# zuston/TonY

Measured on AMD Instinct MI355X. Metric: images/sec (whole node) Inception-v3 TF-PS, higher is better.
Workload: dtype bf16

## Files before the change

### tony_amd/ops/_lib.py

```python
from __future__ import annotations

import ctypes
import os
import threading
import weakref
from typing import Dict

import torch

_HERE = os.path.dirname(os.path.abspath(__file__))
SO_PATH = os.environ.get("TONY_KERNELS_SO") or os.path.join(_HERE, "_tony_kernels.so")

_lock = threading.Lock()
_lib = None

c_void_p = ctypes.c_void_p
c_int = ctypes.c_int
c_int64 = ctypes.c_int64
c_float = ctypes.c_float
c_int_p = ctypes.POINTER(ctypes.c_int)
c_void_pp = ctypes.POINTER(ctypes.c_void_p)
c_u8_p = ctypes.POINTER(ctypes.c_uint8)
c_u64_p = ctypes.POINTER(ctypes.c_uint64)

# ... 20 lines not shown
                               c_void_p, c_int64, c_int64, c_int64, c_int64, c_void_p, c_int64, c_int64, c_int,
                               c_void_p, c_void_p, c_void_p, c_void_p, c_int, c_int, c_void_p, c_void_p, c_int64,
                               c_void_p, c_void_p, c_int, c_void_p],
    "tony_bn_relu_maxpool": [c_void_p, c_int64, c_void_p, c_void_p, c_int64, c_void_p, c_void_p, c_int, c_float,
                             c_void_p, c_void_p, c_void_p, c_void_p, c_float, c_void_p, c_int64, c_void_p, c_int,
                             c_int, c_int, c_int, c_int, c_int, c_int, c_void_p],
    "tony_bn_bwd_reduce": [c_void_p, c_int64, c_void_p, c_int64, c_int64, c_int, c_void_p, c_void_p, c_void_p,
                           c_void_p, c_int, c_int, c_void_p, c_void_p, c_int64, c_void_p],
    "tony_bn_bwd_apply": [c_void_p, c_int64, c_void_p, c_int64, c_void_p, c_int64, c_int64, c_int, c_void_p,
                          c_void_p, c_void_p, c_void_p, c_int, c_int, c_void_p, c_void_p, c_int64, c_void_p,
                          c_void_p, c_int, c_void_p],
    "tony_bn_apply_f32_x3": [c_void_p, c_int64, c_int, c_int64, c_void_p, c_int64, c_void_p, c_void_p, c_int64,
                             c_void_p, c_void_p, c_int, c_float, c_int, c_int, c_void_p, c_void_p, c_void_p, c_void_p,
                             c_float, c_void_p],
    "tony_bn_apply_res": [c_void_p, c_int64, c_int, c_int64, c_void_p, c_int64, c_void_p, c_int64, c_void_p,
                          c_void_p, c_int64, c_void_p, c_void_p, c_int, c_float, c_int, c_int, c_void_p, c_void_p,
                          c_void_p, c_void_p, c_float, c_void_p],
    "tony_bn_apply_res_m": [c_void_p, c_int64, c_int, c_int64, c_void_p, c_int64, c_void_p, c_int64, c_void_p,
                            c_void_p, c_int64, c_void_p, c_void_p, c_int, c_float, c_int, c_int, c_void_p, c_void_p,
                            c_void_p, c_void_p, c_float, c_void_p, c_int64, c_void_p],
    "tony_bn_bwd_res": [c_void_p, c_int64, c_void_p, c_int64, c_void_p, c_int64, c_void_p, c_int64, c_void_p, c_int64,
                        c_int64, c_int, c_void_p, c_void_p, c_void_p, c_void_p, c_int, c_void_p, c_void_p, c_void_p,
                        c_int, c_void_p],
    "tony_bn_bwd_res_m": [c_void_p, c_int64, c_void_p, c_int64, c_void_p, c_int64, c_void_p, c_int64, c_void_p,
                          c_int64, c_int64, c_int, c_void_p, c_void_p, c_void_p, c_void_p, c_int, c_void_p, c_void_p,
                          c_void_p, c_int, c_void_p],
    "tony_bn_bwd_onepass": [c_void_p, c_int64, c_void_p, c_int64, c_void_p, c_int64, c_int64, c_int, c_void_p,
                            c_void_p, c_void_p, c_void_p, c_int, c_int, c_void_p, c_void_p, c_void_p, c_int,
                            c_void_p, c_int, c_void_p],
    "tony_add_f32": [c_void_p, c_int, c_void_p, c_int64, c_void_p],
    "tony_sgd_step": [c_void_p, c_void_p, c_void_p, c_int, c_void_p, c_int64, c_void_p, c_void_p],
    "tony_adam_step": [c_void_p, c_void_p, c_void_p, c_void_p, c_int, c_void_p, c_int64, c_void_p, c_void_p],
    "tony_grad_stats": [c_void_p, c_int, c_int64, c_void_p, c_void_p],
    "tony_xent_fwd": [c_void_p, c_int, c_int64, c_int, c_int64, c_void_p, c_float, c_void_p, c_void_p, c_void_p],
    "tony_xent_bwd": [c_void_p, c_int, c_int64, c_int, c_int64, c_void_p, c_float, c_void_p, c_void_p, c_void_p,
                      c_int64, c_void_p],
    "tony_dropout_fwd": [c_void_p, c_void_p, c_void_p, c_int64, c_int, c_float, c_void_p, c_void_p],
    "tony_dropout_bwd": [c_void_p, c_void_p, c_void_p, c_int64, c_int, c_float, c_void_p],
    "tony_counter_bump": [c_void_p, c_void_p],
    "tony_gemm_bf16": [c_void_p, c_void_p, c_void_p, c_int64, c_int64, c_int64, c_int64, c_int64, c_int64,
                       c_int, c_void_p, c_int64, c_void_p],
    "tony_gemm_bf16_bnact": [c_void_p, c_void_p, c_void_p, c_int64, c_int64, c_int64, c_int64, c_int64, c_int64,
                             c_int, c_void_p, c_int64, c_void_p, c_void_p],
    "tony_gemm_tn_bf16": [c_void_p, c_void_p, c_void_p, c_int64, c_int64, c_int64, c_int64, c_int64, c_int64,
                          c_void_p, c_int64, c_void_p, c_int, c_void_p, c_void_p, c_int, c_void_p],
    "tony_splitk_reduce": [c_void_p, c_int, c_int64, c_void_p, c_int, c_int, c_int, c_void_p],
    "tony_splitk_workspace": [c_void_p, c_int64, c_void_p, c_int64],
    "tony_conv_fwd": [c_void_p, c_int, c_int, c_int, c_int, c_int64, c_void_p, c_int, c_int, c_int, c_int, c_int,
                      c_int, c_int, c_void_p, c_int, c_int, c_int64, c_int, c_void_p, c_int64, c_void_p],
    "tony_stem_fwd": [c_void_p, c_int, c_int, c_int, c_int, c_void_p, c_int, c_int, c_int, c_int, c_int, c_int,
                      c_int, c_void_p, c_int, c_int, c_int64, c_int, c_void_p, c_int64, c_int, c_void_p],
    "tony_stem_wgrad": [c_void_p, c_int64, c_void_p, c_int, c_int, c_int, c_int, c_int, c_int, c_int, c_int, c_int,
                        c_int, c_int, c_int, c_int, c_void_p, c_int64, c_void_p, c_int, c_void_p],
    "tony_conv_dgrad": [c_void_p, c_int, c_int, c_int, c_int, c_int64, c_void_p, c_int, c_int, c_int, c_int, c_int,
                        c_void_p, c_int, c_int, c_int64, c_int, c_void_p, c_void_p],
    "tony_conv_dgrad_strided": [c_void_p, c_int, c_int, c_int, c_int, c_int64, c_void_p, c_int, c_int, c_int, c_int,
                                c_int, c_int, c_int, c_void_p, c_int, c_int, c_int64, c_int, c_void_p, c_void_p],
    "tony_conv_wgrad": [c_void_p, c_int64, c_void_p, c_int, c_int, c_int, c_int, c_int64, c_int, c_int, c_int, c_int,
                        c_int, c_int, c_int, c_int, c_int, c_void_p, c_void_p, c_int64, c_void_p, c_int, c_void_p,
                        c_void_p, c_int, c_void_p],
    "tony_conv_wgrad_x3": [c_void_p, c_int64, c_void_p, c_int, c_int, c_int, c_int, c_int64, c_int, c_int, c_int,
                           c_int, c_int, c_int, c_int, c_int, c_int, c_int, c_int, c_void_p, c_int64, c_void_p, c_int,
                           c_void_p],
    "tony_x3_wgrad_mode": [c_int],
    "tony_dgrad_one_launch": [c_int],
    "tony_wgrad_pf": [c_int],
    "tony_kv_copy_blocks": [c_int64],
    "tony_kv_copy_flag": [c_void_p, c_void_p, c_int64, c_void_p, c_void_p],
    "tony_kv_wait": [c_void_p, ctypes.c_uint32, c_void_p, ctypes.c_double, c_void_p],
    "tony_conv_wgrad_direct": [c_void_p, c_int64, c_void_p, c_int, c_int, c_int, c_int, c_int64, c_int, c_int, c_int,
                               c_int, c_int, c_void_p, c_int64, c_void_p, c_int, c_void_p],
    "tony_avgpool3_s1p1": [c_void_p, c_void_p, c_int, c_int, c_int, c_int, c_int64, c_int64, c_void_p],
    "tony_maxpool_fwd": [c_void_p, c_void_p, c_void_p, c_int, c_int, c_int, c_int, c_int, c_int, c_int, c_int64, c_int64,
                         c_void_p],
    "tony_maxpool_bwd": [c_void_p, c_void_p, c_void_p, c_int, c_int, c_int, c_int, c_int, c_int, c_int, c_int64, c_int64,
                         c_void_p],
    "tony_bn_bwd_pool_apply": [c_void_p, c_int64, c_void_p, c_int, c_int, c_int, c_int, c_int, c_int, c_int, c_void_p,
                               c_int64, c_void_p, c_int64, c_void_p, c_void_p, c_void_p, c_void_p, c_int, c_int,
                               c_void_p, c_int64, c_void_p, c_void_p, c_int, c_void_p],
    "tony_maxpool_bwd_acc": [c_void_p, c_void_p, c_void_p, c_int, c_int, c_int, c_int, c_int, c_int, c_int, c_int64, c_int64,
                         c_void_p],
    "tony_maxpool_bwd_bnred": [c_void_p, c_void_p, c_void_p, c_int, c_int, c_int, c_int, c_int, c_int, c_int, c_int64,
                               c_int64, c_void_p, c_int64, c_void_p, c_void_p, c_void_p, c_void_p, c_int, c_int,
                               c_void_p, c_int64, c_int, c_void_p],
    "tony_avgpool_fwd": [c_void_p, c_void_p, c_int, c_int, c_int, c_int, c_int, c_int, c_int64, c_int64, c_void_p],
    "tony_avgpool_bwd": [c_void_p, c_void_p, c_int, c_int, c_int, c_int, c_int, c_int, c_int64, c_int64, c_void_p],
    "tony_transpose_desc_bytes": [],
    "tony_x3_desc_bytes": [],
    "tony_x3_weights_batch": [c_void_p, c_int, c_int, c_void_p],
    "tony_transpose_batch": [c_void_p, c_int, c_int, c_void_p],
    "tony_event_pool": [c_int, c_u64_p],
    "tony_fork": [c_void_p, c_void_p, c_void_p],
    "tony_bn_stats_f32": [c_void_p, c_int64, c_int, c_int64, c_void_p, c_void_p, c_int64, c_void_p],
    "tony_bn_apply_f32": [c_void_p, c_int64, c_int, c_int64, c_void_p, c_int64, c_void_p, c_void_p, c_int64, c_void_p,
                      c_void_p, c_int, c_float, c_int, c_int, c_void_p, c_void_p, c_void_p, c_void_p, c_float,
                      c_void_p],
    "tony_bn_bwd_reduce_f32": [c_void_p, c_int64, c_void_p, c_int64, c_int64, c_int, c_void_p, c_void_p, c_void_p,
                           c_void_p, c_int, c_int, c_void_p, c_void_p, c_int64, c_void_p],
    "tony_bn_bwd_apply_f32": [c_void_p, c_int64, c_void_p, c_int64, c_void_p, c_int64, c_int64, c_int, c_void_p,
                          c_void_p, c_void_p, c_void_p, c_int, c_int, c_void_p, c_void_p, c_int64, c_void_p,
                          c_void_p, c_int, c_void_p],
    "tony_bn_bwd_apply_f32_x3": [c_void_p, c_int64, c_void_p, c_int64, c_void_p, c_int64, c_int64, c_int, c_void_p,
                          c_void_p, c_void_p, c_void_p, c_int, c_int, c_void_p, c_void_p, c_int64, c_void_p,
                          c_void_p, c_int, c_void_p],
    "tony_bn_bwd_apply_f32_x3p": [c_void_p, c_int64, c_void_p, c_int64, c_void_p, c_int64, c_int64, c_int64, c_int,
                                  c_void_p, c_void_p, c_void_p, c_void_p, c_int, c_int, c_void_p, c_void_p, c_int64,
# ... 286 lines not shown
```

### tony_amd/ops/conv.py

```python
from __future__ import annotations

import ctypes
import os
import weakref
from typing import Callable, Dict, Tuple

import torch

from . import _lib, concat, streams, tape, tune, wt_cache
from .arena import zeros_f32
from .bn import HOST_MEMO, _accum_ok, _as_rows, _rows_view
from .gemm import occ_choices, splitk_combine, wgrad_cus, wgrad_tn

_BF16 = torch.bfloat16
AUTOTUNE = os.environ.get("TONY_CONV_AUTOTUNE", "1") != "0"
_CHOICE: Dict[Tuple, str] = {}


def _pair(v):
    if type(v) is tuple:
        return v
    return tuple(v) if isinstance(v, (tuple, list)) else (int(v), int(v))


# ... 77 lines not shown
            return y
    if x.shape[1] < 8:
        return stem_fwd(x, weight, stride, padding, stats)
    key0 = (x.shape, x.stride(), x.dtype, x.device, weight.shape, weight.stride(), weight.dtype, stride, padding,
            stats is not None)
    x, (_, C, ldx) = _as_rows(x)
    n, _, h, w = x.shape
    co, _, r, s = weight.shape
    _lib.check_stat_buffer(stats, co)
    (sh, sw), (ph, pw) = _pair(stride), _pair(padding)
    oh, ow = out_hw(h, w, r, s, stride, padding)
    y = _cl_empty(n, co, oh, ow, x.device)
    wk = _krsc(weight)
    L, st = _lib.lib(), _lib.stream_ptr(x.device)

    def launch(vf, stats_t):
        return L.tony_conv_fwd(x.data_ptr(), n, h, w, C, ldx, wk.data_ptr(), co, r, s, sh, sw, ph, pw, y.data_ptr(),
                               oh, ow, co, (1 if stats_t is not None else 0) | vf, _lib.ptr(stats_t), 2 * co, st)

    if vflags is None:
        key = ("conv_fwd", tuple(x.shape), ldx, tuple(weight.shape), (sh, sw), (ph, pw), stats is not None)
        vflags = tune.cached(key)
        if vflags is None:
            scratch = torch.zeros(_lib.stat_floats(co), device=x.device) if stats is not None else None
            vflags = tune.pick(key, lambda vf: launch(vf, scratch), tune.CONV_VARIANTS)
        if (HOST_MEMO and key0[1] == x.stride() and x.dtype == _BF16 and weight.dtype == _BF16
                and not torch.cuda.is_current_stream_capturing()):
            _FWD_PLAN[key0] = (n, h, w, C, ldx, co, r, s, sh, sw, ph, pw, oh, ow, vflags)
    _lib.check(launch(vflags, stats), "tony_conv_fwd")
    return y


_FWD_PLAN: Dict[Tuple, Tuple] = {}


def stem_fwd(x: torch.Tensor, weight: torch.Tensor, stride=1, padding=0, stats: torch.Tensor | None = None):
    if not stem_supported(x, weight, stride, padding):
        raise ValueError(f"stem_fwd: unsupported conv x={tuple(x.shape)} w={tuple(weight.shape)}")
    n, c, h, w = x.shape
    co, _, r, s = weight.shape
    _lib.check_stat_buffer(stats, co)
    (sh, sw), (ph, pw) = _pair(stride), _pair(padding)
    oh, ow = out_hw(h, w, r, s, stride, padding)
    y = _cl_empty(n, co, oh, ow, x.device)
    wk = _krsc(weight)
    rc = _lib.lib().tony_stem_fwd(x.data_ptr(), n, h, w, c, wk.data_ptr(), co, r, s, sh, sw, ph, pw, y.data_ptr(),
                                  oh, ow, co, 1 if stats is not None else 0, _lib.ptr(stats),
                                  2 * co if stats is not None else 0, _lib.num_cus(x.device),
                                  _lib.stream_ptr(x.device))
    _lib.check(rc, "tony_stem_fwd")
    return y


def stem_wgrad(dy: torch.Tensor, x: torch.Tensor, weight_shape, stride=1, padding=0, dst=None):
    dy, (_, co, lddy) = _as_rows(dy)
    n, c, h, w = x.shape
    _, _, r, s = weight_shape
    (sh, sw), (ph, pw) = _pair(stride), _pair(padding)
    L, dev = _lib.lib(), x.device
    cus = _lib.num_cus(dev)
    nel = co * r * s * c
    slab = torch.empty(2 * cus * nel, dtype=torch.float32, device=dev)
    splits = ctypes.c_int(0)
    st = _lib.stream_ptr(dev)
    rc = L.tony_stem_wgrad(dy.data_ptr(), lddy, x.data_ptr(), n, h, w, c, co, r, s, sh, sw, ph, pw, dy.shape[2],
                           dy.shape[3], slab.data_ptr(), slab.numel(), ctypes.addressof(splits), cus, st)
    _lib.check(rc, "tony_stem_wgrad")
    out = dst if dst is not None else torch.empty(nel, dtype=torch.float32, device=dev)
    rc = L.tony_splitk_reduce(slab.data_ptr(), splits.value, nel, out.data_ptr(), int(out.dtype == _BF16),
                              int(dst is not None), cus, st)
    _lib.check(rc, "tony_splitk_reduce")
    return None if dst is not None else out.view(co, r, s, c).permute(0, 3, 1, 2)


STRIDED_GLDS = os.environ.get("TONY_STRIDED_GLDS", "1") != "0"


def dgrad_supported(x_shape, weight: torch.Tensor, stride=1, padding=0) -> bool:
    (sh, sw), (ph, pw) = _pair(stride), _pair(padding)
    r, s = weight.shape[2], weight.shape[3]
    return x_shape[1] % 8 == 0 and 1 <= sh <= 4 and 1 <= sw <= 4 and 0 <= ph < r and 0 <= pw < s


def conv_dgrad(dy: torch.Tensor, weight: torch.Tensor, x_shape, stride=1, padding=0,
               vflags: int | None = None, bnr: "_lib.BnRed | None" = None,
               accum: torch.Tensor | None = None) -> torch.Tensor:
    if not dgrad_supported(x_shape, weight, stride, padding):
        raise ValueError(f"conv_dgrad: unsupported x={tuple(x_shape)} w={tuple(weight.shape)} stride={stride} "
                         f"padding={padding}")
    n, c, h, w = x_shape
    co, _, r, s = weight.shape
    dy, (_, _, lddy) = _as_rows(dy)
    (sh, sw), (ph, pw) = _pair(stride), _pair(padding)
    dx = _cl_empty(n, c, h, w, dy.device)
    wt = wt_cache.transposed(weight)
    L, st = _lib.lib(), _lib.stream_ptr(dy.device)

    if (sh, sw) == (1, 1):
        def launch(vf, br=None):
            return L.tony_conv_dgrad(dy.data_ptr(), n, dy.shape[2], dy.shape[3], co, lddy, wt.data_ptr(), c, r, s, ph,
                                     pw, dx.data_ptr(), h, w, c, vf, None if br is None else ctypes.addressof(br), st)
        name = "tony_conv_dgrad"
    else:
        def launch(vf, br=None):
            if (vf >> 8) & 0xff in (9, 10, tune.BAND_CODE):
                return -3
            if not STRIDED_GLDS and (vf >> 8) & 0xff >= 11:
                return -3
            return L.tony_conv_dgrad_strided(dy.data_ptr(), n, dy.shape[2], dy.shape[3], co, lddy, wt.data_ptr(), c,
                                             r, s, sh, sw, ph, pw, dx.data_ptr(), h, w, c, vf,
                                             None if br is None else ctypes.addressof(br), st)
        name = "tony_conv_dgrad_strided"

    vf = vflags if vflags is not None else tune.pick(("conv_dgrad", tuple(dy.shape), lddy, tuple(weight.shape),
                                                         (sh, sw), (ph, pw)), launch, tune.CONV_VARIANTS)
    if accum is not None and bnr is None and _accum_ok(accum, x_shape):
        dx = accum
        rc = launch(vf | 16)
        if rc == -3 and (vf >> 8) & 0xff in (9, 10, tune.BAND_CODE):
            rc = launch((vf & ~0xfff00) | 16)
# ... 260 lines not shown
    impl = _choose(key, cands)
    return conv_dgrad(dy, weight, x_shape, stride, padding, bnr=bnr) if impl == "tony" else \
        _miopen_dgrad(dy, weight, x_shape, stride, padding)


MIOPEN_WGRAD_WEIGHT = float(os.environ.get("TONY_MIOPEN_WGRAD_WEIGHT", "1.6"))
WGRAD_IMPL = os.environ.get("TONY_WGRAD_IMPL", "")


def _wgrad(dy, x, weight, stride, padding):
    key = ("wgrad", tuple(dy.shape), tuple(weight.shape), stride, padding)
    impl = _CHOICE.get(key) or WGRAD_IMPL or None
    if fullcover(x.shape, weight.shape, stride, padding):
        impl = "gemm"
        _CHOICE.setdefault(key, impl)
    elif x.shape[1] % 8:
        impl = "stem" if STEM and stem_supported(x, weight, stride, padding) else "miopen"
        _CHOICE.setdefault(key, impl)
    if impl is None:
        impl = _choose(key, {"tony": lambda: conv_wgrad(dy, x, weight.shape, stride, padding),
                             "miopen": lambda: _miopen_wgrad(dy, x, weight, stride, padding)},
                       weight={"miopen": MIOPEN_WGRAD_WEIGHT if streams.ENABLED else 1.0})
    gw = _lib.grad_slot(weight)
    if impl == "gemm":
        if gw is not None and gw.is_contiguous(memory_format=torch.channels_last):
            return streams.run(lambda: _gemm_wgrad(dy, x, weight.shape, dst=gw), dy, x)
        return _accumulate_wgrad(weight, _gemm_wgrad(dy, x, weight.shape))
    if impl == "stem":
        if gw is not None and gw.is_contiguous(memory_format=torch.channels_last):
            return streams.run(lambda: stem_wgrad(dy, x, weight.shape, stride, padding, dst=gw), dy, x)
        return _accumulate_wgrad(weight, stem_wgrad(dy, x, weight.shape, stride, padding))
    if impl == "tony":
        if gw is not None and gw.is_contiguous(memory_format=torch.channels_last):
            return streams.run(lambda: conv_wgrad(dy, x, weight.shape, stride, padding, dst=gw), dy, x)
        return _accumulate_wgrad(weight, conv_wgrad(dy, x, weight.shape, stride, padding))
    if gw is None:
        return _miopen_wgrad(dy, x, weight, stride, padding)

    def into_slot():
        gw.add_(_miopen_wgrad(dy, x, weight, stride, padding))

    return streams.run(into_slot, dy, x)


def _accumulate_wgrad(weight, dw32):
    gw = _lib.grad_slot(weight)
    if gw is None:
        return dw32.to(weight.dtype)
    src = dw32 if gw.is_contiguous(memory_format=torch.channels_last) else dw32.contiguous()
    rc = _lib.lib().tony_add_f32(gw.data_ptr(), int(gw.dtype == _BF16), src.data_ptr(), src.numel(),
                                 _lib.stream_ptr(weight.device))
    _lib.check(rc, "tony_add_f32")
    return None


class _ConvFn(torch.autograd.Function):
    @staticmethod
    def forward(ctx, x, weight, stride, padding):
        y = _fwd(x, weight, stride, padding, None)
        ctx.save_for_backward(x, weight)
        ctx.params = (weight,)
        ctx.stride, ctx.padding = stride, padding
        ctx.bnc_in = getattr(x, "_tony_bnr", None)
        return y

    @staticmethod
    def backward(ctx, dy):
        x, weight = ctx.saved_tensors
        dy = _as_rows(dy)[0]
        dw = _wgrad(dy, x, weight, ctx.stride, ctx.padding)
        dx = _dgrad_fused_bn(ctx, dy, weight, x.shape, ctx.stride, ctx.padding) if ctx.needs_input_grad[0] else None
        streams.keep(dx)
        _lib.report_inplace(ctx.params, (dw,))
        return dx, dw, None, None


def conv2d(x, weight, stride=1, padding=0):
    if supported(x, weight, stride, padding):
        return tape.apply(_ConvFn, x, weight, _pair(stride), _pair(padding))
    if x.is_cuda:
        _record_unsupported("fwd", x.shape, weight.shape, stride, padding)
    return torch.nn.functional.conv2d(x, weight, None, stride, padding)


class _ConvBNActFn(torch.autograd.Function):

    @staticmethod
    def forward(ctx, x, weight, gamma, beta, running_mean, running_var, stride, padding, training, momentum, eps,
                relu, slot=None):
        L = _lib.lib()
        _lib.check_f32_stats(running_mean, running_var)
        dev = x.device
        stream = _lib.stream_ptr(dev)
        co = weight.shape[0]
        stats = zeros_f32(_lib.stat_floats(co), dev) if training else None
        Z = _fwd(x, weight, stride, padding, stats)
        M, _, ldz = _rows_view(Z)
        y = concat.take(slot, *Z.shape, Z)
        if y is None:
            y = torch.empty_like(Z)
        _, _, ldy = _rows_view(y)
        pb = int(gamma.dtype == _BF16)
        if training:
            mean = torch.empty(co, dtype=torch.float32, device=dev)
            invstd = torch.empty(co, dtype=torch.float32, device=dev)
        else:
            mean = running_mean
            invstd = torch.rsqrt(running_var.float() + eps)
        rc = L.tony_bn_apply(Z.data_ptr(), M, co, ldz, y.data_ptr(), ldy, _lib.ptr(stats),
                             _lib.ptr(stats) + 4 * co if training else 0, 2 * co if training else 0,
                             gamma.data_ptr(), beta.data_ptr(), pb,
                             float(eps), int(relu), 0 if training else 1, _lib.ptr(mean) if training else 0,
                             _lib.ptr(invstd) if training else 0, _lib.ptr(running_mean), _lib.ptr(running_var),
                             float(momentum), stream)
        _lib.check(rc, "tony_bn_apply")
        ctx.save_for_backward(x, weight, gamma, beta, mean, invstd, Z)
        ctx.params = (weight, gamma, beta)
        ctx.cfg = (stride, padding, relu, pb)
        ctx.bnc_in = getattr(x, "_tony_bnr", None)
        ctx.join = getattr(x, "_tony_join", None)
        ctx.bnc_self = None
        if training and slot is None:
            ctx.bnc_self = BnCtx(Z, ldz, mean, invstd, gamma, beta, pb, relu)
            y._tony_bnr = ctx.bnc_self
        return y

    @staticmethod
    def backward(ctx, dy):
        x, weight, gamma, beta, mean, invstd, Z = ctx.saved_tensors
        dx, dw, dgamma, dbeta = _conv_bn_backward(ctx, x, weight, gamma, beta, mean, invstd, Z, dy)
        return dx, dw, dgamma, dbeta, None, None, None, None, None, None, None, None, None


def _bn_grad_slots(ctx, gamma, beta):
    gg, gb = _lib.grad_slot(ctx.params[1]), _lib.grad_slot(ctx.params[2])
    inplace = gg is not None and gb is not None
    return (gg if inplace else torch.empty_like(gamma)), (gb if inplace else torch.empty_like(beta)), inplace


def _conv_bn_backward(ctx, x, weight, gamma, beta, mean, invstd, Z, dy, presums=None, done=None):
    stride, padding, relu, pb = ctx.cfg
    dev = x.device
    if done is not None:
        dZ, dgamma, dbeta, inplace = done
    else:
        M, co, ldz = _rows_view(Z)
        if presums is None:
            presums = _bn_presums(ctx, dy)
        dy, (_, _, lddy) = _as_rows(dy)
        dZ = torch.empty_like(Z)
        ws = None if presums is not None else zeros_f32(_lib.bn_bwd_ws_floats(co), dev)
        dgamma, dbeta, inplace = _bn_grad_slots(ctx, gamma, beta)
        _lib.bn_bwd(Z, ldz, dy, lddy, dZ, ldz, M, co, mean, invstd, gamma, beta, pb, relu, ws, dgamma, dbeta, inplace,
                    dev, sums=presums)
    dw = _wgrad(dZ, x, weight, stride, padding)
    join = getattr(ctx, "join", None) if ctx.needs_input_grad[0] else None
    pend = join.take() if join is not None else None
    if pend is not None:
        dx = _dgrad(dZ, weight, x.shape, stride, padding, accum=pend)
    else:
        dx = _dgrad_fused_bn(ctx, dZ, weight, x.shape, stride, padding) if ctx.needs_input_grad[0] else None
        if join is not None:
            dx = join.settle(dx)
    streams.keep(dx)
    if inplace:
        dgamma = dbeta = None
    _lib.report_inplace(ctx.params, (dw, dgamma, dbeta))
    return dx, dw, dgamma, dbeta


class _ConvBNActPoolFn(torch.autograd.Function):

    @staticmethod
    def forward(ctx, x, weight, gamma, beta, running_mean, running_var, stride, padding, momentum, eps, k, s, p=0):
        L = _lib.lib()
        _lib.check_f32_stats(running_mean, running_var)
        dev = x.device
        co = weight.shape[0]
        stats = zeros_f32(_lib.stat_floats(co), dev)
        Z = _fwd(x, weight, stride, padding, stats)
        _, _, ldz = _rows_view(Z)
        n, _, h, w = Z.shape
        oh, ow = (h + 2 * p - k) // s + 1, (w + 2 * p - k) // s + 1
        y = _cl_empty(n, co, oh, ow, dev)
        arg = torch.empty((n, oh, ow, co), dtype=torch.uint8, device=dev)
        mean = torch.empty(co, dtype=torch.float32, device=dev)
        invstd = torch.empty(co, dtype=torch.float32, device=dev)
        pb = int(gamma.dtype == _BF16)
        rc = L.tony_bn_relu_maxpool(Z.data_ptr(), ldz, stats.data_ptr(), stats.data_ptr() + 4 * co, 2 * co,
                                    gamma.data_ptr(), beta.data_ptr(), pb, float(eps), mean.data_ptr(),
                                    invstd.data_ptr(), _lib.ptr(running_mean), _lib.ptr(running_var), float(momentum),
                                    y.data_ptr(), co, arg.data_ptr(), n, h, w, co, k, s, p, _lib.stream_ptr(dev))
        _lib.check(rc, "tony_bn_relu_maxpool")
        ctx.save_for_backward(x, weight, gamma, beta, mean, invstd, Z, arg)
        ctx.params = (weight, gamma, beta)
        ctx.cfg = (stride, padding, True, pb)
        ctx.pool = (k, s, p)
        ctx.bnc_in = getattr(x, "_tony_bnr", None)
        return y

    @staticmethod
    def backward(ctx, dyp):
        x, weight, gamma, beta, mean, invstd, Z, arg = ctx.saved_tensors
        k, s, p = ctx.pool
        n, co, h, w = Z.shape
# ... 101 lines not shown
```

### tony_amd/ops/csrc/bn_act.hip

```cpp
#include <algorithm>
#include <cstdlib>

#include "common.h"

using namespace tony;

namespace {

constexpr int kThreads = 256;
constexpr int kMaxC = 2048;
extern __shared__ __attribute__((aligned(16))) float bn_dyn[];
inline size_t bn_lds_table(int C, int rows) { return static_cast<size_t>(rows) * C * sizeof(float); }
inline size_t bn_lds_reduce(int C) {
  return static_cast<size_t>(2) * (kThreads / (C / 8)) * C * sizeof(float);
}
inline size_t bn_lds_bred(int C) { return std::max(bn_lds_table(C, 4), bn_lds_reduce(C)); }

struct RowMap {
  int CG, RPI, cg, rsub;
  bool active;
  __device__ RowMap(int C) {
    CG = C >> 3;
    RPI = kThreads / CG;
    cg = threadIdx.x % CG;
    rsub = threadIdx.x / CG;
    active = rsub < RPI;
  }
};

struct Segs {
  int n = 0;
  int end[4] = {0, 0, 0, 0};
  void* p[4] = {nullptr, nullptr, nullptr, nullptr};
  int64_t ld[4] = {0, 0, 0, 0};
  template <class T>
  __device__ __forceinline__ void resolve(int col, T*& base, int64_t& ld_out) const {
    int s = 0, start = 0;
    while (s + 1 < n && col >= end[s]) {
      start = end[s];
      ++s;
    }
    base = static_cast<T*>(p[s]) + (col - start);
    ld_out = ld[s];
  }
};

__device__ __forceinline__ float load_param(const void* p, int idx, int is_bf16, float dflt) {
  if (p == nullptr) return dflt;
  return is_bf16 ? bf2f(static_cast<const uint16_t*>(p)[idx]) : static_cast<const float*>(p)[idx];
}

__device__ __forceinline__ void store_param(void* p, int idx, int is_bf16, float v, int accumulate) {
  if (p == nullptr) return;
  if (is_bf16) {
    uint16_t* q = static_cast<uint16_t*>(p) + idx;
    *q = f2bf(accumulate ? bf2f(*q) + v : v);
  } else {
    float* q = static_cast<float*>(p) + idx;
    *q = accumulate ? *q + v : v;
  }
}

__device__ __forceinline__ void block_reduce_add(float* red, const RowMap& rm, int C,
                                                 const float* a, const float* b, float* out_a, float* out_b) {
  if (rm.active) {
#pragma unroll
    for (int j = 0; j < 8; ++j) {
      red[rm.rsub * C + rm.cg * 8 + j] = a[j];
      red[rm.RPI * C + rm.rsub * C + rm.cg * 8 + j] = b[j];
    }
  }
  __syncthreads();
  for (int c = threadIdx.x; c < C; c += kThreads) {
    float sa = 0.f, sb = 0.f;
    for (int k = 0; k < rm.RPI; ++k) {
      sa += red[k * C + c];
      sb += red[rm.RPI * C + k * C + c];
    }
    atomicAdd(out_a + c, sa);
    atomicAdd(out_b + c, sb);
  }
}

template <class T>
__global__ __launch_bounds__(kThreads) void bn_fwd_stats_kernel(
    const T* __restrict__ x, int64_t M, int C, int64_t ldx, int64_t rows_per_block,
    float* __restrict__ sum, float* __restrict__ sumsq, int64_t sstride) {
  float* red = bn_dyn;
  RowMap rm(C);
  float s[8], q[8];
#pragma unroll
  for (int j = 0; j < 8; ++j) s[j] = q[j] = 0.f;
  const int64_t r0 = static_cast<int64_t>(blockIdx.x) * rows_per_block;
  const int64_t r1 = min(M, r0 + rows_per_block);
  if (rm.active) {
    const T* base = x + rm.cg * 8;
    int64_t r = r0 + rm.rsub;
    const int64_t step = rm.RPI;
    for (; r + 3 * step < r1; r += 4 * step) {
      V8<T> v[4];
#pragma unroll
      for (int u = 0; u < 4; ++u) v[u] = V8<T>::load(base + (r + u * step) * ldx);
#pragma unroll
      for (int u = 0; u < 4; ++u) {
        float f[8];
        v[u].to_float(f);
#pragma unroll
        for (int j = 0; j < 8; ++j) {
          s[j] += f[j];
          q[j] = fmaf(f[j], f[j], q[j]);
        }
      }
    }
    for (; r < r1; r += step) {
// ... 1113 lines not shown
```

### tony_amd/ops/csrc/common.h

```cpp
#pragma once
#include <hip/hip_runtime.h>
#include <stdint.h>

#define TONY_API extern "C" __attribute__((visibility("default")))

namespace tony {

static constexpr int kWave = 64;

static constexpr int kStatShards = 8;

__device__ __forceinline__ float shard_sum(const float* p, int c, int64_t sstride) {
  if (sstride == 0) return p[c];
  float s = 0.f;
#pragma unroll
  for (int k = 0; k < kStatShards; ++k) s += p[k * sstride + c];
  return s;
}

__device__ __forceinline__ int64_t shard_off(int idx, int64_t sstride) {
  return sstride == 0 ? 0 : static_cast<int64_t>(idx % kStatShards) * sstride;
}

__device__ __forceinline__ float relu_f(float t) { return t < 0.f ? 0.f : t; }

__device__ __forceinline__ float bf2f(uint16_t v) {
  return __uint_as_float(static_cast<uint32_t>(v) << 16);
}

__device__ __forceinline__ uint16_t f2bf(float f) {
  __bf16 b = static_cast<__bf16>(f);
  return __builtin_bit_cast(uint16_t, b);
}

struct bf16x8 {
  uint4 raw;
  __device__ __forceinline__ void to_float(float* f) const {
    const uint32_t w[4] = {raw.x, raw.y, raw.z, raw.w};
#pragma unroll
    for (int i = 0; i < 4; ++i) {
      f[2 * i] = __uint_as_float(w[i] << 16);
      f[2 * i + 1] = __uint_as_float(w[i] & 0xffff0000u);
    }
  }
  __device__ __forceinline__ static bf16x8 from_float(const float* f) {
    bf16x8 r;
    uint32_t w[4];
#pragma unroll
    for (int i = 0; i < 4; ++i) {
      w[i] = static_cast<uint32_t>(f2bf(f[2 * i])) |
             (static_cast<uint32_t>(f2bf(f[2 * i + 1])) << 16);
    }
    r.raw = make_uint4(w[0], w[1], w[2], w[3]);
    return r;
  }
};

__device__ __forceinline__ bf16x8 load8(const uint16_t* p) {
  bf16x8 r;
  r.raw = *reinterpret_cast<const uint4*>(p);
  return r;
}
__device__ __forceinline__ void store8(uint16_t* p, const bf16x8& v) {
  *reinterpret_cast<uint4*>(p) = v.raw;
}

template <class T>
struct V8;
template <>
struct V8<uint16_t> {
  bf16x8 b;
  __device__ __forceinline__ static V8 load(const uint16_t* p) { return V8{load8(p)}; }
  __device__ __forceinline__ void store(uint16_t* p) const { store8(p, b); }
  __device__ __forceinline__ void to_float(float* f) const { b.to_float(f); }
  __device__ __forceinline__ static V8 from_float(const float* f) { return V8{bf16x8::from_float(f)}; }
};
template <>
struct V8<float> {
  float4 lo, hi;
  __device__ __forceinline__ static V8 load(const float* p) {
    return V8{*reinterpret_cast<const float4*>(p), *reinterpret_cast<const float4*>(p + 4)};
  }
  __device__ __forceinline__ void store(float* p) const {
    *reinterpret_cast<float4*>(p) = lo;
    *reinterpret_cast<float4*>(p + 4) = hi;
// ... 30 lines not shown
```

### tony_amd/ops/csrc/stem.hip

```cpp
#include <type_traits>
#include "mfma_common.h"

using namespace tony;
using namespace tony::mfma;

namespace {

constexpr int kBM = 256;
constexpr int kPatch = 12288;
constexpr int kPF = kPatch / 8 / kThreads;
constexpr int kMaxKSteps = 8;

struct StemGeom {
  const uint16_t* x;
  int H, W, C;
  int R, S, sh, sw, ph, pw;
  int OH, OW;
  int M;
  int K;
  int64_t total;
  float inv_ohw, inv_ow;
};

__device__ __forceinline__ int fast_div(int a, int b, float inv_b) {
// ... 168 lines not shown
#pragma unroll
        for (int i = 0; i < TM; ++i) {
          uint16_t v[8];
#pragma unroll
          for (int e = 0; e < 8; ++e) v[e] = tap_value<NP>(g, src, px[i], tp[e]);
          const bf16x8_t af = pack8(v);
#pragma unroll
          for (int j = 0; j < TN; ++j)
            acc[i][j] = __builtin_amdgcn_mfma_f32_16x16x32_bf16(af, bfr[j], acc[i][j], 0, 0, 0);
        }
      }
    };
    if (staged)
      body(smem);
    else
      body(g.x);
    __syncthreads();
#pragma unroll
    for (int j = 0; j < TN; ++j)
#pragma unroll
      for (int i = 0; i < TM; ++i)
#pragma unroll
        for (int r = 0; r < 4; ++r) {
          const float a = acc[i][j][r];
          ssum[j] += a;
          ssq[j] = fmaf(a, a, ssq[j]);
          smem[(wave * 64 + i * 16 + kq * 4 + r) * LDC + j * 16 + (lane & 15)] = f2bf(a);
        }
    __syncthreads();
    constexpr int CH = BN / 8;
    for (int v = threadIdx.x; v < kBM * CH; v += kThreads) {
      const int row = v / CH, ch = v - row * CH;
      if (m0 + row < g.M)
        *reinterpret_cast<uint4*>(y + static_cast<int64_t>(m0 + row) * ldy + ch * 8) =
            *reinterpret_cast<const uint4*>(smem + row * LDC + ch * 8);
    }
  }
  if (stats == nullptr) return;
  float* st = stats + shard_off(blockIdx.x, sstride);
#pragma unroll
  for (int j = 0; j < TN; ++j) {
    float a = ssum[j], q = ssq[j];
    a += __shfl_xor(a, 16, 64);
    a += __shfl_xor(a, 32, 64);
    q += __shfl_xor(q, 16, 64);
    q += __shfl_xor(q, 32, 64);
    if (lane < 16) {
      atomicAdd(st + j * 16 + lane, a);
      atomicAdd(st + BN + j * 16 + lane, q);
    }
  }
}

template <int CO, int KB, bool NP>
__global__ __launch_bounds__(kThreads) void stem_wgrad_kernel(StemGeom g, const uint16_t* __restrict__ dy,
                                                              int64_t lddy, float* __restrict__ slab, int64_t n) {
  constexpr int PD = CO + 4;
  constexpr int CB = CO / 16;
  constexpr int KW = KB * 16;
  constexpr int DYL = kBM * PD;
  constexpr int RED = CO * KW;
  constexpr int DV = kBM * CO / 8 / kThreads;
  static_assert(RED * 4 <= (DYL + kPatch) * 2, "the fold tile reuses the staging buffers");
  __shared__ __attribute__((aligned(16))) uint16_t smem[DYL + kPatch];
  uint16_t* dyl = smem;
  uint16_t* patch = smem + DYL;

  const int lane = threadIdx.x & 63, wave = threadIdx.x >> 6;
  const int kq = lane >> 4;
  const int kcol0 = blockIdx.y * KW;
  const int kbn = min(KB, (g.K - kcol0 + 15) / 16);
  uint32_t tp[KB];
#pragma unroll
  for (int b = 0; b < KB; ++b) tp[b] = tap_word(g, kcol0 + b * 16 + (lane & 15));

  f32x4 acc[CB][KB];
#pragma unroll
  for (int i = 0; i < CB; ++i)
#pragma unroll
    for (int j = 0; j < KB; ++j) acc[i][j] = f32x4{0.f, 0.f, 0.f, 0.f};

  const int nchunks = (g.M + kBM - 1) / kBM;
  RowPrefetch pf;
  uint4 dv[DV];
  auto issue = [&](int chunk) {
    const int m0 = chunk * kBM, rows = min(kBM, g.M - m0);
    pf.issue(g, m0, m0 + rows - 1);
#pragma unroll
    for (int i = 0; i < DV; ++i) {
      const int v = i * kThreads + threadIdx.x, r = v / (CO / 8), c8 = v % (CO / 8);
      dv[i] = r < rows ? *reinterpret_cast<const uint4*>(dy + static_cast<int64_t>(m0 + r) * lddy + c8 * 8)
                       : make_uint4(0u, 0u, 0u, 0u);
    }
  };
  if (blockIdx.x < nchunks) issue(blockIdx.x);
  for (int chunk = blockIdx.x; chunk < nchunks; chunk += gridDim.x) {
    const int m0 = chunk * kBM;
    __syncthreads();
#pragma unroll
    for (int i = 0; i < DV; ++i) {
      const int v = i * kThreads + threadIdx.x, r = v / (CO / 8), c8 = v % (CO / 8);
      uint2* d = reinterpret_cast<uint2*>(dyl + r * PD + c8 * 8);
      d[0] = make_uint2(dv[i].x, dv[i].y);
      d[1] = make_uint2(dv[i].z, dv[i].w);
    }
    pf.commit(patch);
    const bool staged = pf.staged;
    const int64_t e0 = staged ? pf.e0 : 0;
    __syncthreads();
    if (chunk + static_cast<int>(gridDim.x) < nchunks) issue(chunk + gridDim.x);
    auto body = [&](const uint16_t* src) {
#pragma unroll
      for (int step = 0; step < 2; ++step) {
        const int p0 = wave * 64 + step * 32 + kq * 8;
        bf16x8_t af[CB];
#pragma unroll
        for (int i = 0; i < CB; ++i) {
          uint16_t v[8];
#pragma unroll
          for (int e = 0; e < 8; ++e) v[e] = dyl[(p0 + e) * PD + i * 16 + (lane & 15)];
          af[i] = pack8(v);
        }
        Pix px[8];
        px[0].init(g, m0 + p0, e0);
#pragma unroll
        for (int e = 1; e < 8; ++e) {
          px[e] = px[e - 1];
          px[e].next(g, m0 + p0 + e, e0);
        }
#pragma unroll
        for (int j = 0; j < KB; ++j) {
          if (j >= kbn) break;
          uint16_t v[8];
#pragma unroll
          for (int e = 0; e < 8; ++e) v[e] = tap_value<NP>(g, src, px[e], tp[j]);
          const bf16x8_t bfr = pack8(v);
#pragma unroll
          for (int i = 0; i < CB; ++i)
            acc[i][j] = __builtin_amdgcn_mfma_f32_16x16x32_bf16(af[i], bfr, acc[i][j], 0, 0, 0);
        }
      }
    };
    if (staged)
      body(patch);
    else
      body(g.x);
  }

  __syncthreads();
  float* red = reinterpret_cast<float*>(smem);
  for (int v = threadIdx.x; v < RED; v += kThreads) red[v] = 0.f;
  __syncthreads();
#pragma unroll
  for (int i = 0; i < CB; ++i)
// ... 44 lines not shown
    const int stage = kPatch > kBM * (bn + 8) ? kPatch : kBM * (bn + 8);
    return static_cast<size_t>(stage + ksteps * (bn / 16) * 64 * 8) * sizeof(uint16_t);
  };
  static int occ_cache[2][kMaxKSteps + 1];
  auto grid_for = [&](const void* fn, size_t bytes) {
    int& per_cu = occ_cache[Co == 64][ksteps];
    if (per_cu <= 0 &&
        (hipOccupancyMaxActiveBlocksPerMultiprocessor(&per_cu, fn, kThreads, bytes) != hipSuccess || per_cu <= 0))
      per_cu = 2;
    return min(ceil_div(g.M, kBM), per_cu * (num_cus > 0 ? num_cus : 256));
  };
  const bool np = ph == 0 && pw == 0;
  const auto launch = [&](auto bn_c, auto np_c) {
    constexpr int BN = decltype(bn_c)::value;
    constexpr bool NP = decltype(np_c)::value;
    const size_t b = lds(BN);
    stem_fwd_kernel<BN, NP><<<grid_for(reinterpret_cast<const void*>(&stem_fwd_kernel<BN, NP>), b), kThreads, b,
                               stream>>>(g, static_cast<const uint16_t*>(w), static_cast<uint16_t*>(y), ldy, st, sstride);
  };
  using std::integral_constant;
  if (Co == 32)
    np ? launch(integral_constant<int, 32>{}, std::true_type{}) : launch(integral_constant<int, 32>{}, std::false_type{});
  else
    np ? launch(integral_constant<int, 64>{}, std::true_type{}) : launch(integral_constant<int, 64>{}, std::false_type{});
  TONY_LAUNCH_CHECK();
  return 0;
}

TONY_API int tony_stem_wgrad(const void* dy, int64_t lddy, const void* x, int N, int H, int W, int C, int Co, int R,
                             int S, int sh, int sw, int ph, int pw, int OH, int OW, float* slab, int64_t slab_cap,
                             int* splits, int num_cus, hipStream_t stream) {
  StemGeom g;
  if (!make_geom(g, x, N, H, W, C, Co, R, S, sh, sw, ph, pw, OH, OW)) return -1;
  if (dy == nullptr || slab == nullptr || splits == nullptr || num_cus <= 0 || lddy < Co || (lddy % 8) ||
      (reinterpret_cast<uintptr_t>(dy) & 15))
    return -1;
  const int64_t n = static_cast<int64_t>(Co) * g.K;
  const int nchunks = ceil_div(g.M, kBM);
  const bool k5 = Co == 64 && g.K > 64 && g.K <= 160;
  static int occ[3] = {0, 0, 0};
  const int which = k5 ? 2 : (Co == 64);
  if (occ[which] == 0) {
    const void* fn = k5 ? reinterpret_cast<const void*>(&stem_wgrad_kernel<64, 5, false>)
                        : Co == 64 ? reinterpret_cast<const void*>(&stem_wgrad_kernel<64, 4, false>)
                                   : reinterpret_cast<const void*>(&stem_wgrad_kernel<32, 4, false>);
    if (hipOccupancyMaxActiveBlocksPerMultiprocessor(&occ[which], fn, kThreads, 0) != hipSuccess || occ[which] <= 0)
      occ[which] = 1;
  }
  const int gx = min(nchunks, min(2, occ[which]) * num_cus);
  if (static_cast<int64_t>(gx) * n > slab_cap) return -1;
  const bool np = ph == 0 && pw == 0;
  const auto launch = [&](auto co_c, auto kb_c, auto np_c, int gy) {
    stem_wgrad_kernel<decltype(co_c)::value, decltype(kb_c)::value, decltype(np_c)::value>
        <<<dim3(gx, gy), kThreads, 0, stream>>>(g, static_cast<const uint16_t*>(dy), lddy, slab, n);
  };
  using std::integral_constant;
  using I4 = integral_constant<int, 4>;
  if (k5)
    np ? launch(integral_constant<int, 64>{}, integral_constant<int, 5>{}, std::true_type{}, ceil_div(g.K, 80))
       : launch(integral_constant<int, 64>{}, integral_constant<int, 5>{}, std::false_type{}, ceil_div(g.K, 80));
  else if (Co == 32)
    np ? launch(integral_constant<int, 32>{}, I4{}, std::true_type{}, ceil_div(g.K, 64))
       : launch(integral_constant<int, 32>{}, I4{}, std::false_type{}, ceil_div(g.K, 64));
  else
    np ? launch(integral_constant<int, 64>{}, I4{}, std::true_type{}, ceil_div(g.K, 64))
       : launch(integral_constant<int, 64>{}, I4{}, std::false_type{}, ceil_div(g.K, 64));
  TONY_LAUNCH_CHECK();
  *splits = gx;
  return 0;
}
```

Measured before the change: 9714.

## Fuse BN-backward elementwise into stem conv weight-gradient kernel

When the first (stem) conv needs no input gradient, the batch-norm backward elementwise step is folded into the stem wgrad kernel. The kernel loads Z with dy, applies the ReLU mask and BN affine correction in registers, and stages the result for the wgrad MMA. This avoids writing and rereading a full dZ tensor and saves a launch. The cost is extra per-element arithmetic and Z loads inside the wgrad kernel, plus more shared memory, which may lower occupancy.

Result: no change. 9749, median of 5 (+0.4%).

```diff
diff --git a/tony_amd/ops/_lib.py b/tony_amd/ops/_lib.py
--- a/tony_amd/ops/_lib.py
+++ b/tony_amd/ops/_lib.py
@@ -96,6 +96,10 @@
                       c_int, c_void_p, c_int, c_int, c_int64, c_int, c_void_p, c_int64, c_int, c_void_p],
     "tony_stem_wgrad": [c_void_p, c_int64, c_void_p, c_int, c_int, c_int, c_int, c_int, c_int, c_int, c_int, c_int,
                         c_int, c_int, c_int, c_int, c_void_p, c_int64, c_void_p, c_int, c_void_p],
+    "tony_stem_wgrad_bn": [c_void_p, c_int64, c_void_p, c_int64, c_void_p, c_int, c_int, c_int, c_int, c_int, c_int,
+                           c_int, c_int, c_int, c_int, c_int, c_int, c_int, c_void_p, c_void_p, c_void_p, c_void_p,
+                           c_int, c_int, c_void_p, c_void_p, c_int64, c_void_p, c_void_p, c_int, c_void_p, c_int64,
+                           c_void_p, c_int, c_void_p],
     "tony_conv_dgrad": [c_void_p, c_int, c_int, c_int, c_int, c_int64, c_void_p, c_int, c_int, c_int, c_int, c_int,
                         c_void_p, c_int, c_int, c_int64, c_int, c_void_p, c_void_p],
     "tony_conv_dgrad_strided": [c_void_p, c_int, c_int, c_int, c_int, c_int64, c_void_p, c_int, c_int, c_int, c_int,
diff --git a/tony_amd/ops/conv.py b/tony_amd/ops/conv.py
--- a/tony_amd/ops/conv.py
+++ b/tony_amd/ops/conv.py
@@ -153,7 +153,25 @@
     return y
 
 
-def stem_wgrad(dy: torch.Tensor, x: torch.Tensor, weight_shape, stride=1, padding=0, dst=None):
+STEM_FUSE = os.environ.get("TONY_STEM_FUSE", "1") != "0"
+STEM_FUSE_HITS = [0]
+
+
+class StemBnBwd:
+    __slots__ = ("Z", "ldz", "mean", "invstd", "gamma", "beta", "pb", "relu", "sums", "dgamma", "dbeta", "accumulate")
+
+    def __init__(self, Z, ldz, mean, invstd, gamma, beta, pb, relu, sums, dgamma, dbeta, accumulate):
+        self.Z, self.ldz, self.mean, self.invstd, self.gamma, self.beta = Z, ldz, mean, invstd, gamma, beta
+        self.pb, self.relu, self.sums = int(pb), int(relu), sums
+        self.dgamma, self.dbeta, self.accumulate = dgamma, dbeta, bool(accumulate)
+
+
+def stem_wgrad_bn_supported(x: torch.Tensor, weight: torch.Tensor, stride=1, padding=0) -> bool:
+    return (stem_supported(x, weight, stride, padding) and weight.shape[0] == 32
+            and weight.shape[1] * weight.shape[2] * weight.shape[3] <= 64)
+
+
+def stem_wgrad(dy: torch.Tensor, x: torch.Tensor, weight_shape, stride=1, padding=0, dst=None, bn=None):
     dy, (_, co, lddy) = _as_rows(dy)
     n, c, h, w = x.shape
     _, _, r, s = weight_shape
@@ -164,9 +182,17 @@
     slab = torch.empty(2 * cus * nel, dtype=torch.float32, device=dev)
     splits = ctypes.c_int(0)
     st = _lib.stream_ptr(dev)
-    rc = L.tony_stem_wgrad(dy.data_ptr(), lddy, x.data_ptr(), n, h, w, c, co, r, s, sh, sw, ph, pw, dy.shape[2],
-                           dy.shape[3], slab.data_ptr(), slab.numel(), ctypes.addressof(splits), cus, st)
-    _lib.check(rc, "tony_stem_wgrad")
+    if bn is not None:
+        rc = L.tony_stem_wgrad_bn(dy.data_ptr(), lddy, bn.Z.data_ptr(), bn.ldz, x.data_ptr(), n, h, w, c, co, r, s,
+                                  sh, sw, ph, pw, dy.shape[2], dy.shape[3], bn.mean.data_ptr(), bn.invstd.data_ptr(),
+                                  _lib.ptr(bn.gamma), _lib.ptr(bn.beta), bn.pb, bn.relu, bn.sums.data_ptr(),
+                                  bn.sums.data_ptr() + 4 * co, 2 * co, _lib.ptr(bn.dgamma), _lib.ptr(bn.dbeta),
+                                  int(bn.accumulate), slab.data_ptr(), slab.numel(), ctypes.addressof(splits), cus, st)
+        _lib.check(rc, "tony_stem_wgrad_bn")
+    else:
+        rc = L.tony_stem_wgrad(dy.data_ptr(), lddy, x.data_ptr(), n, h, w, c, co, r, s, sh, sw, ph, pw, dy.shape[2],
+                               dy.shape[3], slab.data_ptr(), slab.numel(), ctypes.addressof(splits), cus, st)
+        _lib.check(rc, "tony_stem_wgrad")
     out = dst if dst is not None else torch.empty(nel, dtype=torch.float32, device=dev)
     rc = L.tony_splitk_reduce(slab.data_ptr(), splits.value, nel, out.data_ptr(), int(out.dtype == _BF16),
                               int(dst is not None), cus, st)
@@ -533,6 +559,27 @@
                                  _lib.stream_ptr(weight.device))
     _lib.check(rc, "tony_add_f32")
     return None
+
+
+def _stem_wgrad_bn(weight, x, stride, padding, dy, lddy, bn: StemBnBwd, reduce: bool):
+    if reduce:
+        M, co, _ = _rows_view(bn.Z)
+        rc = _lib.lib().tony_bn_bwd_reduce(bn.Z.data_ptr(), bn.ldz, dy.data_ptr(), lddy, M, co, bn.mean.data_ptr(),
+                                           bn.invstd.data_ptr(), _lib.ptr(bn.gamma), _lib.ptr(bn.beta), bn.pb,
+                                           bn.relu, bn.sums.data_ptr(), bn.sums.data_ptr() + 4 * co, 2 * co,
+                                           _lib.stream_ptr(x.device))
+        _lib.check(rc, "tony_bn_bwd_reduce")
+    STEM_FUSE_HITS[0] += 1
+    _CHOICE.setdefault(("wgrad", tuple(dy.shape), tuple(weight.shape), stride, padding), "stem")
+    gw = _lib.grad_slot(weight)
+    if gw is not None and gw.is_contiguous(memory_format=torch.channels_last):
+        def into_slot():
+            return stem_wgrad(dy, x, weight.shape, stride, padding, dst=gw, bn=bn)
+
+        if bn.accumulate:
+            return streams.run(into_slot, dy, bn.Z, x, bn.sums, bn.mean, bn.invstd)
+        return into_slot()
+    return _accumulate_wgrad(weight, stem_wgrad(dy, x, weight.shape, stride, padding, bn=bn))
 
 
 class _ConvFn(torch.autograd.Function):
@@ -629,9 +676,18 @@
         if presums is None:
             presums = _bn_presums(ctx, dy)
         dy, (_, _, lddy) = _as_rows(dy)
-        dZ = torch.empty_like(Z)
         ws = None if presums is not None else zeros_f32(_lib.bn_bwd_ws_floats(co), dev)
         dgamma, dbeta, inplace = _bn_grad_slots(ctx, gamma, beta)
+        if (STEM_FUSE and STEM and not ctx.needs_input_grad[0]
+                and stem_wgrad_bn_supported(x, weight, stride, padding)):
+            dw = _stem_wgrad_bn(weight, x, stride, padding, dy, lddy,
+                                StemBnBwd(Z, ldz, mean, invstd, gamma, beta, pb, relu, presums if ws is None else ws,
+                                          dgamma, dbeta, inplace), reduce=ws is not None)
+            if inplace:
+                dgamma = dbeta = None
+            _lib.report_inplace(ctx.params, (dw, dgamma, dbeta))
+            return None, dw, dgamma, dbeta
+        dZ = torch.empty_like(Z)
         _lib.bn_bwd(Z, ldz, dy, lddy, dZ, ldz, M, co, mean, invstd, gamma, beta, pb, relu, ws, dgamma, dbeta, inplace,
                     dev, sums=presums)
     dw = _wgrad(dZ, x, weight, stride, padding)
diff --git a/tony_amd/ops/csrc/bn_act.hip b/tony_amd/ops/csrc/bn_act.hip
--- a/tony_amd/ops/csrc/bn_act.hip
+++ b/tony_amd/ops/csrc/bn_act.hip
@@ -44,22 +44,6 @@
     ld_out = ld[s];
   }
 };
-
-__device__ __forceinline__ float load_param(const void* p, int idx, int is_bf16, float dflt) {
-  if (p == nullptr) return dflt;
-  return is_bf16 ? bf2f(static_cast<const uint16_t*>(p)[idx]) : static_cast<const float*>(p)[idx];
-}
-
-__device__ __forceinline__ void store_param(void* p, int idx, int is_bf16, float v, int accumulate) {
-  if (p == nullptr) return;
-  if (is_bf16) {
-    uint16_t* q = static_cast<uint16_t*>(p) + idx;
-    *q = f2bf(accumulate ? bf2f(*q) + v : v);
-  } else {
-    float* q = static_cast<float*>(p) + idx;
-    *q = accumulate ? *q + v : v;
-  }
-}
 
 __device__ __forceinline__ void block_reduce_add(float* red, const RowMap& rm, int C,
                                                  const float* a, const float* b, float* out_a, float* out_b) {
diff --git a/tony_amd/ops/csrc/common.h b/tony_amd/ops/csrc/common.h
--- a/tony_amd/ops/csrc/common.h
+++ b/tony_amd/ops/csrc/common.h
@@ -31,6 +31,22 @@
 __device__ __forceinline__ uint16_t f2bf(float f) {
   __bf16 b = static_cast<__bf16>(f);
   return __builtin_bit_cast(uint16_t, b);
+}
+
+__device__ __forceinline__ float load_param(const void* p, int idx, int is_bf16, float dflt) {
+  if (p == nullptr) return dflt;
+  return is_bf16 ? bf2f(static_cast<const uint16_t*>(p)[idx]) : static_cast<const float*>(p)[idx];
+}
+
+__device__ __forceinline__ void store_param(void* p, int idx, int is_bf16, float v, int accumulate) {
+  if (p == nullptr) return;
+  if (is_bf16) {
+    uint16_t* q = static_cast<uint16_t*>(p) + idx;
+    *q = f2bf(accumulate ? bf2f(*q) + v : v);
+  } else {
+    float* q = static_cast<float*>(p) + idx;
+    *q = accumulate ? *q + v : v;
+  }
 }
 
 struct bf16x8 {
diff --git a/tony_amd/ops/csrc/stem.hip b/tony_amd/ops/csrc/stem.hip
--- a/tony_amd/ops/csrc/stem.hip
+++ b/tony_amd/ops/csrc/stem.hip
@@ -244,9 +244,22 @@
   }
 }
 
-template <int CO, int KB, bool NP>
+struct BnBwdOp {
+  const uint16_t* z;
+  int64_t ldz;
+  const float *mean, *invstd;
+  const void *gamma, *beta;
+  const float *dsum, *dsumx;
+  int64_t sstride;
+  void *dgamma, *dbeta;
+  int param_bf16, relu, accumulate;
+};
+struct NoBnBwd {};
+
+template <int CO, int KB, bool NP, bool FUSE = false>
 __global__ __launch_bounds__(kThreads) void stem_wgrad_kernel(StemGeom g, const uint16_t* __restrict__ dy,
-                                                              int64_t lddy, float* __restrict__ slab, int64_t n) {
+                                                              int64_t lddy, float* __restrict__ slab, int64_t n,
+                                                              std::conditional_t<FUSE, BnBwdOp, NoBnBwd> f) {
   constexpr int PD = CO + 4;
   constexpr int CB = CO / 16;
   constexpr int KW = KB * 16;
@@ -254,7 +267,7 @@
   constexpr int RED = CO * KW;
   constexpr int DV = kBM * CO / 8 / kThreads;
   static_assert(RED * 4 <= (DYL + kPatch) * 2, "the fold tile reuses the staging buffers");
-  __shared__ __attribute__((aligned(16))) uint16_t smem[DYL + kPatch];
+  __shared__ __attribute__((aligned(16))) uint16_t smem[DYL + kPatch + (FUSE ? 10 * CO : 0)];
   uint16_t* dyl = smem;
   uint16_t* patch = smem + DYL;
 
@@ -275,6 +288,7 @@
   const int nchunks = (g.M + kBM - 1) / kBM;
   RowPrefetch pf;
   uint4 dv[DV];
+  uint4 zv[FUSE ? DV : 1];
   auto issue = [&](int chunk) {
     const int m0 = chunk * kBM, rows = min(kBM, g.M - m0);
     pf.issue(g, m0, m0 + rows - 1);
@@ -283,15 +297,60 @@
       const int v = i * kThreads + threadIdx.x, r = v / (CO / 8), c8 = v % (CO / 8);
       dv[i] = r < rows ? *reinterpret_cast<const uint4*>(dy + static_cast<int64_t>(m0 + r) * lddy + c8 * 8)
                        : make_uint4(0u, 0u, 0u, 0u);
+      if constexpr (FUSE)
+        zv[i] = r < rows ? *reinterpret_cast<const uint4*>(f.z + static_cast<int64_t>(m0 + r) * f.ldz + c8 * 8)
+                         : make_uint4(0u, 0u, 0u, 0u);
     }
   };
   if (blockIdx.x < nchunks) issue(blockIdx.x);
+  float* tab = reinterpret_cast<float*>(smem + DYL + kPatch);
+  if constexpr (FUSE) {
+    static_assert(kThreads % (CO / 8) == 0, "a thread's channel group is the same in every piece");
+    const float inv_m = 1.f / static_cast<float>(g.M);
+    for (int c = threadIdx.x; c < CO; c += kThreads) {
+      const float ga = load_param(f.gamma, c, f.param_bf16, 1.f), be = load_param(f.beta, c, f.param_bf16, 0.f);
+      const float ds = shard_sum(f.dsum, c, f.sstride), dsx = shard_sum(f.dsumx, c, f.sstride);
+      const float mu = f.mean[c], is = f.invstd[c];
+      const float k = ga * is, am = ds * inv_m, bm = dsx * inv_m;
+      tab[0 * CO + c] = k;
+      tab[1 * CO + c] = -k * bm * is;
+      tab[2 * CO + c] = k * (bm * is * mu - am);
+      tab[3 * CO + c] = k;
+      tab[4 * CO + c] = be - k * mu;
+      if (blockIdx.x == 0 && blockIdx.y == 0) {
+        store_param(f.dbeta, c, f.param_bf16, ds, f.accumulate);
+        store_param(f.dgamma, c, f.param_bf16, dsx, f.accumulate);
+      }
+    }
+  }
   for (int chunk = blockIdx.x; chunk < nchunks; chunk += gridDim.x) {
     const int m0 = chunk * kBM;
     __syncthreads();
+    float q[FUSE ? 5 : 1][8];
+    if constexpr (FUSE) {
+      const int c0 = threadIdx.x % (CO / 8) * 8;
+#pragma unroll
+      for (int t = 0; t < 5; ++t)
+#pragma unroll
+        for (int j = 0; j < 8; ++j) q[t][j] = tab[t * CO + c0 + j];
+    }
 #pragma unroll
     for (int i = 0; i < DV; ++i) {
       const int v = i * kThreads + threadIdx.x, r = v / (CO / 8), c8 = v % (CO / 8);
+      if constexpr (FUSE) {
+        if (r < g.M - m0) {
+          float xf[8], gf[8], o[8];
+          bf16x8{zv[i]}.to_float(xf);
+          bf16x8{dv[i]}.to_float(gf);
+#pragma unroll
+          for (int j = 0; j < 8; ++j) {
+            float d = gf[j];
+            if (f.relu && fmaf(xf[j], q[3][j], q[4][j]) <= 0.f) d = 0.f;
+            o[j] = fmaf(d, q[0][j], fmaf(xf[j], q[1][j], q[2][j]));
+          }
+          dv[i] = bf16x8::from_float(o).raw;
+        }
+      }
       uint2* d = reinterpret_cast<uint2*>(dyl + r * PD + c8 * 8);
       d[0] = make_uint2(dv[i].x, dv[i].y);
       d[1] = make_uint2(dv[i].z, dv[i].w);
@@ -442,7 +501,7 @@
   const bool np = ph == 0 && pw == 0;
   const auto launch = [&](auto co_c, auto kb_c, auto np_c, int gy) {
     stem_wgrad_kernel<decltype(co_c)::value, decltype(kb_c)::value, decltype(np_c)::value>
-        <<<dim3(gx, gy), kThreads, 0, stream>>>(g, static_cast<const uint16_t*>(dy), lddy, slab, n);
+        <<<dim3(gx, gy), kThreads, 0, stream>>>(g, static_cast<const uint16_t*>(dy), lddy, slab, n, NoBnBwd{});
   };
   using std::integral_constant;
   using I4 = integral_constant<int, 4>;
@@ -459,3 +518,39 @@
   *splits = gx;
   return 0;
 }
+
+TONY_API int tony_stem_wgrad_bn(const void* dy, int64_t lddy, const void* z, int64_t ldz, const void* x, int N, int H,
+                                int W, int C, int Co, int R, int S, int sh, int sw, int ph, int pw, int OH, int OW,
+                                const float* mean, const float* invstd, const void* gamma, const void* beta,
+                                int param_bf16, int relu, const float* dsum, const float* dsumx, int64_t sstride,
+                                void* dgamma, void* dbeta, int accumulate, float* slab, int64_t slab_cap, int* splits,
+                                int num_cus, hipStream_t stream) {
+  StemGeom g;
+  if (Co != 32 || !make_geom(g, x, N, H, W, C, Co, R, S, sh, sw, ph, pw, OH, OW) || g.K > 64) return -1;
+  if (dy == nullptr || z == nullptr || slab == nullptr || splits == nullptr || num_cus <= 0 || lddy < Co ||
+      (lddy % 8) || ldz < Co || (ldz % 8) || ((reinterpret_cast<uintptr_t>(dy) | reinterpret_cast<uintptr_t>(z)) & 15) ||
+      mean == nullptr || invstd == nullptr || dsum == nullptr || dsumx == nullptr || sstride < 0)
+    return -1;
+  const int64_t n = static_cast<int64_t>(Co) * g.K;
+  const bool np = ph == 0 && pw == 0;
+  static int occ[2] = {0, 0};
+  if (occ[np] == 0) {
+    const void* fn = np ? reinterpret_cast<const void*>(&stem_wgrad_kernel<32, 4, true, true>)
+                        : reinterpret_cast<const void*>(&stem_wgrad_kernel<32, 4, false, true>);
+    if (hipOccupancyMaxActiveBlocksPerMultiprocessor(&occ[np], fn, kThreads, 0) != hipSuccess || occ[np] <= 0)
+      occ[np] = 1;
+  }
+  const int gx = min(ceil_div(g.M, kBM), min(2, occ[np]) * num_cus);
+  if (static_cast<int64_t>(gx) * n > slab_cap) return -1;
+  const BnBwdOp f{static_cast<const uint16_t*>(z), ldz, mean, invstd, gamma, beta, dsum, dsumx, sstride, dgamma, dbeta,
+                  param_bf16, relu, accumulate};
+  if (np)
+    stem_wgrad_kernel<32, 4, true, true>
+        <<<dim3(gx, 1), kThreads, 0, stream>>>(g, static_cast<const uint16_t*>(dy), lddy, slab, n, f);
+  else
+    stem_wgrad_kernel<32, 4, false, true>
+        <<<dim3(gx, 1), kThreads, 0, stream>>>(g, static_cast<const uint16_t*>(dy), lddy, slab, n, f);
+  TONY_LAUNCH_CHECK();
+  *splits = gx;
+  return 0;
+}
```
